# alshai/Big-BWT

Measured on AMD Instinct MI355X. Metric: input MB/s to .bwt (bit-exact vs ref), higher is better.
Workload: dtype u8; 1 GPU; BASELINE configs[2]: 64x mutated yeast-shaped FASTA (~0.79 GB), -w 10 -p 100, BWT + -s -e sampled SA; bytes_per_gpu=787308470, w=10, p=100, flags=6, phrases=16409159, words=921010, dict_bytes=79900101, parallelism=1 GPU

## Files before the change

big-bwt_amd/csrc/api_fm.hip:

```cpp
#include <algorithm>
#include <memory>
#include <utility>
#include <vector>
#include "api.hpp"

using namespace pfp;

struct pfp_fm {
  pfp::FmIndex f;
};

namespace {

template <class F>
int dev_call(pfp_fm *fm, F &&body, bool wait = true) {
  pfp_ctx *c = fm->f.c;
  PFP_TRY_DEV(c)
  body();
  if (wait) sync(c);
  return PFP_OK;
  PFP_CATCH(c)
}

template <class T>
T *hand_out(DBuf<T> &b) { return std::exchange(b.p, nullptr); }

template <class F>
int build_call(pfp_ctx *c, pfp_fm **out, F &&build) {
  *out = nullptr;
  PFP_TRY_DEV(c)
  auto fm = std::make_unique<pfp_fm>();
  build(fm->f);
  *out = fm.release();
  return PFP_OK;
  PFP_CATCH(c)
}

uint64_t pattern_bytes(const uint8_t *pat, const uint64_t *pat_off, uint64_t npat) {
  if (!npat) return 0;
  for (uint64_t p = 0; p < npat; p++)
    PFP_REQUIRE(pat_off[p] <= pat_off[p + 1], PFP_EINVAL, "pattern offsets decrease at pattern " + std::to_string(p));
  PFP_REQUIRE(pat || !pat_off[npat], PFP_EINVAL, "no pattern bytes");
  return pat_off[npat];
}

struct HostPatterns {
  DBuf<uint8_t> pat;
  DBuf<uint64_t> off;
// ... 906 lines not shown
```

big-bwt_amd/csrc/chain.hip:

```cpp
#include "chain.hpp"

using namespace pfp;

namespace pfp {

__global__ void occ_lex_kernel(uint32_t d, const uint32_t *__restrict__ lexrank, const uint32_t *__restrict__ wocc,
                               uint32_t *__restrict__ occ_lex, uint32_t *__restrict__ word_at_rank) {
  uint32_t j = BID * blockDim.x + threadIdx.x;
  if (j >= d) return;
  uint32_t r = lexrank[j];
  occ_lex[r] = wocc[j];
  if (word_at_rank) word_at_rank[r] = j;
}
__global__ void parse_sym_kernel(uint64_t P, const uint32_t *__restrict__ pid, const uint32_t *__restrict__ lexrank,
                                 uint32_t *__restrict__ sym) {
  uint64_t k = (uint64_t)BID * blockDim.x + threadIdx.x;
  if (k < P) sym[k] = lexrank[pid[k]] + 1;
}
__global__ __launch_bounds__(256) void dict_permute_kernel(uint32_t d, const uint32_t *__restrict__ word_at_rank,
                                                           const uint64_t *__restrict__ woff,
                                                           const uint32_t *__restrict__ wlen,
                                                           const uint8_t *__restrict__ src,
                                                           const uint64_t *__restrict__ doff, uint8_t *__restrict__ dst) {
  uint64_t t = (uint64_t)BID * 256 + threadIdx.x;
// ... 76 lines not shown
    st.sa_rounds_parse = ch.pb.rounds;
    if (c->debug) validate_parse_bwt(c, ch.pb);
  }
  {
    PhaseTimer t(c, &st.ms_merge);
    BwtOutputs &bo = ch.out;
    if ((flags & PFP_FLAG_SA) && !d_sa) { ch.sa_own.alloc(c, ch.n_used + 1); d_sa = ch.sa_own.p; }
    bo.d_bwt = d_bwt; bo.d_sa = d_sa;
    with_width(ch.ord.wide, [&](auto tag) {
      using I = decltype(tag);
      merge_bwt<I>(c, ch.D, ch.ix, ch.ord.get<I>(), ch.pb, ch.occ_lex.p, MergeOpts::whole(w, flags, ch.n_used + 1), bo);
    });
    st.hard_groups = bo.hard_groups; st.hard_chars = bo.hard_chars;
    st.hard_big_groups = bo.hard_big_groups; st.hard_max_chars = bo.hard_max_chars; st.hard_max_members = bo.hard_max_members;
    st.hard_minor_groups = bo.hard_minor_groups; st.hard_minor_chars = bo.hard_minor_chars;
  }
  sync(c);
  st.ms_total = std::chrono::duration<double, std::milli>(std::chrono::steady_clock::now() - t0).count();
  *n_used = ch.n_used;
}

template <class Sink>
static void emit_outputs(pfp_ctx *c, const uint8_t *d_bwt, const SaView &d_sa, uint64_t n_out, int flags, Sink &&sink) {
  sink("bwt", d_bwt, n_out);
  if (flags & PFP_FLAG_SA) {
    uint64_t cnt = n_out - 1;
    DBuf<uint8_t> packed(c, cnt * 5 + 16);
    PFP_REQUIRE(d_sa.dense, PFP_EINVAL, "full SA output without the SA values");
    pack5_dev(c, d_sa.dense + 1, cnt, packed.p);
    sink("sa", packed.p, cnt * 5);
    sync(c);
  }
  if (flags & PFP_FLAG_SSA) {
    DBuf<uint8_t> pairs;
    uint64_t k = sample_runs_dev(c, d_bwt, d_sa, n_out, false, pairs);
    sink("ssa", pairs.p, k * 10);
    sync(c);
  }
  if (flags & PFP_FLAG_ESA) {
    DBuf<uint8_t> pairs;
    uint64_t k = sample_runs_dev(c, d_bwt, d_sa, n_out, true, pairs);
    sink("esa", pairs.p, k * 10);
    sync(c);
  }
  sync(c);
}
void fetch_outputs(pfp_ctx *c, const uint8_t *d_bwt, const SaView &d_sa, uint64_t n_out, int flags, pfp_bwt_result *out) {
  emit_outputs(c, d_bwt, d_sa, n_out, flags, [&](const char *name, const uint8_t *d, uint64_t bytes) {
    uint8_t *h = fetch_bytes(c, d, bytes);
    if (name[0] == 'b') { out->bwt = h; out->bwt_size = bytes; }
    else if (name[0] == 's' && name[1] == 'a') { out->sa = h; out->sa_bytes = bytes; }
    else if (name[0] == 's') { out->ssa = h; out->ssa_bytes = bytes; }
    else { out->esa = h; out->esa_bytes = bytes; }
  });
}

}

static bool trace_host() { static const bool on = getenv("PFP_TRACE_HOST") != nullptr; return on; }
static std::chrono::steady_clock::time_point now() { return std::chrono::steady_clock::now(); }
static double ms(std::chrono::steady_clock::time_point a, std::chrono::steady_clock::time_point b) { return std::chrono::duration<double, std::milli>(b - a).count(); }

template <class Stage>
static int bigbwt_to_files(pfp_ctx *c, uint64_t n, int w, uint64_t p, int flags, const char *base, uint64_t out_bytes[4], Stage &&stage) {
  PFP_TRY_DEV(c)
  check_args(w, p, flags);
  const auto t0 = now();
  join_background(c);
  MappedOut m_bwt, m_sa;
  const bool map_bwt = m_bwt.start(c, std::string(base) + ".bwt", n + 1);
  const bool map_sa = (flags & PFP_FLAG_SA) && n && m_sa.start(c, std::string(base) + ".sa", n * 5);
  Chain ch;
  stage(ch.tx);
  if (trace_host()) sync(c);
  const auto t1 = now();
  DBuf<uint8_t> d_bwt(c, n + 1 + 16);
  uint64_t used = 0;
  run_chain_dev(c, ch, n, w, p, flags, d_bwt.p, nullptr, &used);
  const auto t2 = now();
  uint64_t sizes[4] = {0, 0, 0, 0};
  int n_mapped = 0;
  emit_outputs(c, d_bwt.p, sa_view(ch.out), used + 1, flags, [&](const char *name, const uint8_t *d, uint64_t bytes) {
    sizes[name[0] == 'b' ? 0 : (name[1] == 'a' ? 1 : (name[0] == 's' ? 2 : 3))] = bytes;
    if (trace_host()) fprintf(stderr, "[pfp]   %.1f ms after the chain: .%s (%.2f GB) is on the device\n", ms(t2, now()), name, bytes / 1e9);
    MappedOut *mo = name[0] == 'b' ? (map_bwt ? &m_bwt : nullptr) : (name[0] == 's' && name[1] == 'a' && name[2] == 0 ? (map_sa ? &m_sa : nullptr) : nullptr);
    MappedOut late;
    if (!mo && late.start(c, std::string(base) + "." + name, bytes)) mo = &late;
    if (mo && mo->active() && bytes <= mo->bytes) {
      if (mo->write(c, d, bytes)) {
        n_mapped++;
        if (mo != &m_bwt) mo->finish(c, bytes);
        return;
      }
      mo->abandon(false);
    } else if (mo && mo->active()) mo->abandon(false);
    write_dev_file(c, std::string(base) + "." + name, 0, d, bytes, true);
  });
  if (trace_host()) fprintf(stderr, "[pfp]   %.1f ms after the chain: the other files are written\n", ms(t2, now()));
  if (m_bwt.active()) m_bwt.finish(c, sizes[0]);
  if (m_sa.active()) m_sa.abandon(true);
  if (trace_host())
    fprintf(stderr, "[pfp] file to files: text in %.1f ms, chain %.1f ms (first call: the pool is cold), files out %.1f ms%s\n", ms(t0, t1), ms(t1, t2),
            ms(t2, now()), n_mapped ? (std::string(" (") + std::to_string(n_mapped) + " of them straight into the files' mapped pages)").c_str() : "");
  if (out_bytes) memcpy(out_bytes, sizes, sizeof sizes);
  return PFP_OK;
// ... 68 lines not shown
  uint64_t used = 0;
  run_chain_dev(c, ch, n, w, p, flags, d_bwt.p, nullptr, &used);
  const auto t2 = now();
  fetch_outputs(c, d_bwt.p, sa_view(ch.out), used + 1, flags, out);
  if (trace_host())
    fprintf(stderr, "[pfp] host boundary: text in %.1f ms, chain %.1f ms, outputs out %.1f ms (%.2f GB in, %.2f GB out)\n", ms(t0, t1), ms(t1, t2),
            ms(t2, now()), n / 1e9, (out->bwt_size + out->sa_bytes + out->ssa_bytes + out->esa_bytes) / 1e9);
  return PFP_OK;
  PFP_CATCH(c)
}

int pfp_bigbwt_formats_dev(pfp_ctx *c, const void *d_text, uint64_t n, int w, uint64_t p, int flags, void *d_bwt,
                           void *d_out[3], uint64_t out_bytes[3], uint64_t *n_used) {
  if (!c || (!d_text && n) || !d_bwt || !d_out || !out_bytes) return PFP_EINVAL;
  for (int k = 0; k < 3; k++) { d_out[k] = nullptr; out_bytes[k] = 0; }
  PFP_TRY_DEV(c)
  check_args(w, p, flags);
  PFP_REQUIRE(((uintptr_t)d_bwt & 15) == 0, PFP_EINVAL, "d_bwt must be 16-byte aligned");
  Chain ch;
  ch.tx.stage(c, d_text, true, n, w);
  uint64_t used = 0;
  run_chain_dev(c, ch, n, w, p, flags, (uint8_t *)d_bwt, nullptr, &used);
  if (n_used) *n_used = used;
  emit_outputs(c, (const uint8_t *)d_bwt, sa_view(ch.out), used + 1, flags, [&](const char *name, const uint8_t *d, uint64_t bytes) {
    if (name[0] == 'b') return;
    const int k = name[1] == 'a' ? 0 : (name[0] == 's' ? 1 : 2);
    hipError_t e = hipSuccess;
    void *q = c->pool.get(bytes ? bytes : 1, &e, __FILE__, __LINE__);
    if (!q) throw Error(PFP_ENOMEM, std::string("device allocation of an output buffer failed: ") + hipGetErrorString(e));
    PFP_HIP(hipMemcpyAsync(q, d, bytes, hipMemcpyDeviceToDevice, c->stream));
    d_out[k] = q; out_bytes[k] = bytes;
  });
  sync(c);
  return PFP_OK;
  PFP_CATCH(c)
}

int pfp_bigbwt_files(pfp_ctx *c, const uint8_t *text, uint64_t n, int w, uint64_t p, int flags, const char *base,
                     uint64_t out_bytes[4]) {
  if (!c || (!text && n) || !base) return PFP_EINVAL;
  return bigbwt_to_files(c, n, w, p, flags, base, out_bytes, [&](StagedText &tx) { tx.stage(c, text, false, n, w); });
}
int pfp_bigbwt_fd(pfp_ctx *c, int fd, uint64_t file_offset, uint64_t n, int w, uint64_t p, int flags, const char *base,
                  uint64_t out_bytes[4]) {
  if (!c || fd < 0 || !base) return PFP_EINVAL;
  return bigbwt_to_files(c, n, w, p, flags, base, out_bytes, [&](StagedText &tx) { tx.stage_fd(c, fd, file_offset, n, w); });
}

}
```

big-bwt_amd/csrc/common.hpp:

```cpp
#pragma once
#include <hip/hip_runtime.h>
#include <cstdint>
#include <cstdio>
#include <cstring>
#include <stdexcept>
#include <string>
#include <vector>
#include <chrono>
#include <map>
#include <thread>
#include "../../include/pfpgpu.h"

struct K1Scratch; struct DistState;
namespace pfp {
struct StagedText;

constexpr uint8_t kDollar = 2, kEndOfWord = 1, kEndOfDict = 0;
constexpr uint32_t kPrime = 1999999973u;

struct Error : std::runtime_error {
  int code;
  Error(int c, const std::string &m) : std::runtime_error(m), code(c) {}
};

#define PFP_HIP(expr)                                                                     \
  do {                                                                                    \
    hipError_t e__ = (expr);                                                              \
    if (e__ != hipSuccess)                                                                \
      throw ::pfp::Error(PFP_EHIP, std::string(#expr) + ": " + hipGetErrorString(e__) +   \
                                       " (" + __FILE__ + ":" + std::to_string(__LINE__) + ")"); \
  } while (0)

#define PFP_REQUIRE(cond, code, msg)                       \
// ... 214 lines not shown
  DBuf(DBuf &&o) noexcept { *this = std::move(o); }
  DBuf &operator=(DBuf &&o) noexcept {
    if (this != &o) { release(); p = o.p; n = o.n; ctx = o.ctx; o.p = nullptr; o.n = 0; }
    return *this;
  }
  ~DBuf() { release(); }
  void alloc(pfp_ctx *c, size_t count, const char *file = __builtin_FILE(), int line = __builtin_LINE()) {
    release();
    ctx = c; n = count;
    size_t bytes = (count ? count : 1) * sizeof(T);
    if (!c->pool.debug) bytes = (bytes + 511) & ~size_t(511);
    hipError_t e;
    p = (T *)c->pool.get(bytes, &e, file, line);
    if (!p)
      throw Error(e == hipErrorOutOfMemory ? PFP_ENOMEM : PFP_EHIP,
                  std::string("hipMalloc(") + std::to_string(bytes) + "): " + hipGetErrorString(e));
  }
  void release() {
    if (p) { ctx->pool.put(p); p = nullptr; n = 0; }
  }
  void zero() { PFP_HIP(hipMemsetAsync(p, 0, n * sizeof(T), ctx->stream)); }
  size_t bytes() const { return n * sizeof(T); }
};

template <class T>
inline void alloc_counts(pfp_ctx *c, DBuf<T> &b, size_t n, size_t pad = 1, const char *file = __builtin_FILE(), int line = __builtin_LINE()) {
  b.alloc(c, n + pad, file, line);
  PFP_HIP(hipMemsetAsync(b.p + n, 0, sizeof(T), c->stream));
}

template <class T>
inline void d2h(pfp_ctx *c, T *dst, const T *src, size_t count) {
  PFP_HIP(hipMemcpyAsync(dst, src, count * sizeof(T), hipMemcpyDeviceToHost, c->stream));
}
template <class T>
inline void h2d(pfp_ctx *c, T *dst, const T *src, size_t count) {
  PFP_HIP(hipMemcpyAsync(dst, src, count * sizeof(T), hipMemcpyHostToDevice, c->stream));
}
inline void sync(pfp_ctx *c) { c->n_syncs++; PFP_HIP(hipStreamSynchronize(c->stream)); }

template <class T>
inline T read_scalar(pfp_ctx *c, const T *dptr) {
  static_assert(sizeof(T) <= 8, "scalar");
  PFP_HIP(hipMemcpyAsync(c->h_scalars, dptr, sizeof(T), hipMemcpyDeviceToHost, c->stream));
  sync(c);
  T v;
// ... 31 lines not shown
```

big-bwt_amd/csrc/kernels.hpp:

```cpp
#pragma once
#include "common.hpp"
#include "wordview.hpp"

namespace pfp {

struct StagedText {
  static constexpr size_t kFront = 64, kBack = 128;
  DBuf<uint8_t> buf;
  uint64_t n = 0;
  int w = 0;
  const uint8_t *tbase() const { return buf.p + kFront; }
  const uint8_t *tprime() const { return buf.p + kFront - 1; }
  void stage(pfp_ctx *c, const void *src, bool src_on_device, uint64_t n_, int w_);
  void stage_fd(pfp_ctx *c, int fd, uint64_t file_off, uint64_t n_, int w_);
  void restage_tail(pfp_ctx *c, uint64_t new_n, int w_) const;
};

struct KRParams {
  static constexpr uint32_t kMaxExtra = 32;
  uint32_t negpw, pinv, pshift, plimit;
  float fdens = 1.0f;
  uint32_t fthr_nom = 0, fauto = 0;
  uint32_t fast = 0, fseed = 0, fthr = 0;
  uint32_t nextra;
  uint64_t bloom;
  uint32_t extra[kMaxExtra];
};
KRParams make_kr_params(int w, uint64_t p);
KRParams make_fast_params(pfp_ctx *c, const StagedText &tx, uint64_t n, int w, uint64_t p);
KRParams make_fast_params_host(const uint8_t *first_window, int w, uint64_t p, double density_setting, double *density_used);
KRParams params_from_plan(int w, uint64_t p, const uint64_t plan[4]);
struct CutSample { DBuf<uint8_t> nominal; DBuf<uint64_t> hashes; uint64_t ns = 0, counted = 0; };
void classify_cuts(pfp_ctx *c, const StagedText &tx, int w, const DBuf<uint64_t> &d_ends, uint64_t ne, const KRParams &kp, uint64_t min_end,
                   CutSample &out);
bool sample_says_dense(pfp_ctx *c, const uint64_t *d_sorted, uint64_t ns, uint64_t p, uint64_t counts[2] = nullptr);
uint64_t keep_nominal_cuts(pfp_ctx *c, DBuf<uint64_t> &d_ends, uint64_t ne, const DBuf<uint8_t> &nominal);
uint32_t window_hash_host(const uint8_t *win, int w, uint32_t seed);
void scan_flags(pfp_ctx *c, const uint8_t *tbase, uint64_t n, int w, uint64_t p, uint16_t *flags16,
                uint32_t *block_counts, unsigned long long *first_bad, const KRParams *kp_override = nullptr);
uint64_t scan_text(pfp_ctx *c, const StagedText &tx, uint64_t n, int w, uint64_t p, DBuf<uint64_t> &d_ends,
                   uint64_t *n_used, const KRParams *kp_override = nullptr);
uint32_t propose_extra_triggers(pfp_ctx *c, const StagedText &tx, uint64_t n_used, int w, uint64_t max_phrase,
                                const DBuf<uint64_t> &d_ends, uint64_t ne, KRParams &kp);
struct ScanReport {
  KRParams first{}, kp{};
  bool chose = false, dense = false, kr_fallback = false;
  uint64_t sampled = 0, kept = 0, distinct = 0, singles = 0;
  std::vector<uint64_t> dense_ends;
  std::vector<uint8_t> nominal;
};
uint64_t scan_text_adaptive(pfp_ctx *c, const StagedText &tx, uint64_t n, int w, uint64_t p, uint64_t max_phrase,
                            DBuf<uint64_t> &d_ends, uint64_t *n_used, uint32_t *n_extra, ScanReport *rep = nullptr);

struct Dictionary {
  uint64_t P = 0;
  uint64_t d = 0;
  uint64_t dsize = 0;
  DBuf<uint8_t> bytes;
  DBuf<uint64_t> woff;
  DBuf<uint32_t> wlen;
  DBuf<uint32_t> wocc;
  DBuf<uint32_t> pid;
  DBuf<uint8_t> last;
  DBuf<uint64_t> sai;
// ... 329 lines not shown
```

big-bwt_amd/csrc/scan.hip:

```cpp
#include "kernels.hpp"
#include "prims.hpp"
#include "devutil.hpp"

namespace pfp {

constexpr uint32_t kBarrettM = 2305843040u;
static_assert((uint64_t)kBarrettM * kPrime <= (1ull << 62), "barrett");
static_assert((uint64_t)(kBarrettM + 1ull) * kPrime > (1ull << 62), "barrett");

template <int S>
__device__ __forceinline__ uint32_t kr_reduce(uint64_t T) {
  uint32_t xs = (uint32_t)(T >> S);
  uint32_t qhat = __umulhi(xs, kBarrettM) >> (30 - S);
  uint32_t r = (uint32_t)T - qhat * kPrime;
  uint32_t r2 = r - kPrime;
  return r < r2 ? r : r2;
}

constexpr uint32_t kB48 = 140737u;
static_assert((uint64_t)kB48 * kPrime <= (1ull << 48) && (uint64_t)(kB48 + 1) * kPrime > (1ull << 48), "barrett48");
__device__ __forceinline__ uint32_t kr_reduce40(uint32_t lo, uint32_t hi) {
  const uint32_t a = __builtin_amdgcn_alignbit(hi, lo, 16) & 0xFFFFFFu;
  const uint32_t qhat = (uint32_t)(((uint64_t)a * (uint64_t)kB48) >> 32) & 0x3FFu;
  const uint32_t prod = __umul24(qhat, kPrime & 0xFFFFu) + (__umul24(qhat, kPrime >> 16) << 16);
// ... 112 lines not shown
template <int W>
__global__ __launch_bounds__(256) void kr_flag_kernel(const uint8_t *__restrict__ tbase, uint64_t n, KRParams kp,
                                                      uint16_t *__restrict__ flags16,
                                                      uint32_t *__restrict__ block_counts,
                                                      unsigned long long *__restrict__ first_bad) {
  const uint64_t c = (uint64_t)BID * 256 + threadIdx.x;
  const uint64_t pos0 = c * 16;
  uint32_t mask = 0;
  if (pos0 < n) {
    mask = kr_mask16<W>(tbase, pos0, n, kp, first_bad);
    flags16[c] = (uint16_t)mask;
  }
  uint32_t cnt = __popc(mask);
#pragma unroll
  for (int off = 32; off > 0; off >>= 1) cnt += __shfl_down(cnt, off, 64);
  __shared__ uint32_t wsum[4];
  if ((threadIdx.x & 63) == 0) wsum[threadIdx.x >> 6] = cnt;
  __syncthreads();
  if (threadIdx.x == 0 && (uint64_t)BID * 4096 < n) block_counts[BID] = wsum[0] + wsum[1] + wsum[2] + wsum[3];
}

constexpr unsigned long long kTagAgg = 1ull << 62, kTagPre = 2ull << 62, kTagMask = 3ull << 62;
constexpr int kScanChunks = 16;
template <int W, bool FAST>
__global__ __launch_bounds__(256) void kr_scan_kernel(const uint8_t *__restrict__ tbase, uint64_t n, KRParams kp, uint64_t ntiles,
                                                      unsigned int *__restrict__ ticket, unsigned long long *__restrict__ state,
                                                      uint64_t *__restrict__ ends, uint64_t cap,
                                                      unsigned long long *__restrict__ first_bad) {
  __shared__ uint32_t wsum[kScanChunks][4];
  __shared__ unsigned int s_tile;
  __shared__ unsigned long long s_excl;
  if (threadIdx.x == 0) s_tile = atomicAdd(ticket, 1u);
  __syncthreads();
  const uint64_t tile = s_tile;
  if (tile >= ntiles) return;
  const int lane = threadIdx.x & 63, wv = threadIdx.x >> 6;
  uint32_t mask[kScanChunks], incl[kScanChunks];
#pragma unroll 1
  for (int j = 0; j < kScanChunks; j++) {
    const uint64_t c0 = (tile * kScanChunks + j) * 4096;
    const uint64_t pos0 = c0 + (uint64_t)threadIdx.x * 16;
    const bool interior = c0 >= 16 && c0 + 4096 <= n;
    mask[j] = pos0 < n ? kr_mask16<W, FAST>(tbase, pos0, n, kp, first_bad, interior) : 0u;
  }
#pragma unroll
  for (int j = 0; j < kScanChunks; j++) {
    const uint32_t v = wave_incl_sum(__popc(mask[j]));
    incl[j] = v;
    if (lane == 63) wsum[j][wv] = v;
  }
  __syncthreads();
// ... 21 lines not shown
      }
      if (lane == 0) __hip_atomic_store(&state[tile], kTagPre | (excl + agg), __ATOMIC_RELAXED, __HIP_MEMORY_SCOPE_AGENT);
    }
    if (lane == 0) s_excl = excl;
  }
  __syncthreads();
  uint64_t chunk_base = s_excl;
#pragma unroll
  for (int j = 0; j < kScanChunks; j++) {
    uint32_t m = mask[j];
    if (m) {
      uint64_t o = chunk_base + (incl[j] - __popc(m));
      for (int q = 0; q < wv; q++) o += wsum[j][q];
      const uint64_t pos0 = ((tile * kScanChunks + j) * 256 + threadIdx.x) * 16;
      while (m) {
        const int b = __ffs(m) - 1;
        m &= m - 1;
        if (o < cap) ends[o] = pos0 + (uint64_t)b;
        o++;
      }
    }
    chunk_base += (uint64_t)wsum[j][0] + wsum[j][1] + wsum[j][2] + wsum[j][3];
  }
}

__global__ __launch_bounds__(256) void kr_flag_generic_kernel(const uint8_t *__restrict__ tbase, uint64_t n, int W,
                                                              KRParams kp, uint16_t *__restrict__ flags16,
                                                              uint32_t *__restrict__ block_counts,
                                                              unsigned long long *__restrict__ first_bad) {
  const uint64_t c = (uint64_t)BID * 256 + threadIdx.x;
  const uint64_t pos0 = c * 16;
  uint32_t mask = 0;
  if (pos0 < n) {
    for (int k = 0; k < 16; k++)
      if (pos0 + k < n && tbase[pos0 + k] <= 2) { atomicMin(first_bad, (unsigned long long)(pos0 + k)); break; }
    uint32_t h = 0;
    if (pos0 + 1 >= (uint64_t)W) {
      for (int k = 0; k < W; k++) h = kr_reduce<8>(((uint64_t)h << 8) | tbase[pos0 - (W - 1) + k]);
      if (kr_divides(h, kp)) mask |= 1u;
    }
    for (int j = 1; j < 16; j++) {
      uint64_t pos = pos0 + j;
      if (pos + 1 < (uint64_t)W) continue;
      if (pos + 1 == (uint64_t)W) {
        h = 0;
        for (int k = 0; k < W; k++) h = kr_reduce<8>(((uint64_t)h << 8) | tbase[k]);
// ... 139 lines not shown
  hipLaunchKernelGGL(kr_flag_kernel<W>, gdim(nblocks), gdim(256), 0, c->stream, tbase, n, kp, flags16, bc, fb);
}

void scan_flags(pfp_ctx *c, const uint8_t *tbase, uint64_t n, int w, uint64_t p, uint16_t *flags16,
                uint32_t *block_counts, unsigned long long *first_bad, const KRParams *kp_override) {
  KRParams kp = kp_override ? *kp_override : make_kr_params(w, p);
  uint64_t nchunks = cdiv64(n, 16);
  int nblocks = (int)cdiv64(nchunks, 256);
  if (nblocks == 0) return;
  KScope ks(c, "pfp::kr_flag_kernel", n + n / 8);
  switch (w) {
#define CASE(W) case W: launch_flag<W>(c, nblocks, tbase, n, kp, flags16, block_counts, first_bad); break;
    CASE(4) CASE(5) CASE(6) CASE(7) CASE(8) CASE(9) CASE(10) CASE(11) CASE(12) CASE(13) CASE(14) CASE(15) CASE(16) CASE(17)
#undef CASE
    default:
      hipLaunchKernelGGL(kr_flag_generic_kernel, gdim(nblocks), gdim(256), 0, c->stream, tbase, n, w, kp, flags16,
                         block_counts, first_bad);
  }
  PFP_HIP(hipGetLastError());
}

template <int W>
static void launch_scan(pfp_ctx *c, uint64_t ntiles, const uint8_t *tbase, uint64_t n, const KRParams &kp, unsigned int *ticket,
                        unsigned long long *state, uint64_t *ends, uint64_t cap, unsigned long long *fb) {
  if (kp.fast) hipLaunchKernelGGL((kr_scan_kernel<W, true>), gdim(ntiles), gdim(256), 0, c->stream, tbase, n, kp, ntiles, ticket, state, ends, cap, fb);
  else hipLaunchKernelGGL((kr_scan_kernel<W, false>), gdim(ntiles), gdim(256), 0, c->stream, tbase, n, kp, ntiles, ticket, state, ends, cap, fb);
}

uint64_t scan_text(pfp_ctx *c, const StagedText &tx, uint64_t n, int w, uint64_t p, DBuf<uint64_t> &d_ends,
                   uint64_t *n_used, const KRParams *kp_override) {
  PFP_REQUIRE(w >= 1 && w <= 4096, PFP_EINVAL, "window size out of range");
  uint64_t cur_n = n;
  uint64_t cap_hint = 0;
  for (int attempt = 0; attempt < 4; attempt++) {
    uint64_t nchunks = cdiv64(cur_n, 16);
    int nblocks = (int)cdiv64(nchunks, 256);
    *n_used = cur_n;
    if (nblocks == 0) { d_ends.alloc(c, 1); return 0; }
    DBuf<unsigned long long> fbad(c, 1);
    PFP_HIP(hipMemsetAsync(fbad.p, 0xff, 8, c->stream));
    if (w >= 4 && w <= 17) {
      const KRParams kp = kp_override ? *kp_override : make_kr_params(w, p);
      const uint64_t ntiles = cdiv64((uint64_t)nblocks, kScanChunks);
      const uint64_t expect = (uint64_t)((double)(cur_n / (p ? p : 1)) * (kp.fast && kp.fdens > 1.0f ? (double)kp.fdens : 1.0));
      const uint64_t cap = cap_hint ? cap_hint : std::min<uint64_t>(cur_n, expect * 4 + 65536);
      d_ends.alloc(c, cap + 1);
      DBuf<unsigned long long> state(c, ntiles);
      DBuf<unsigned int> ticket(c, 1);
      state.zero(); ticket.zero();
      {
        KScope ks(c, "pfp::kr_scan_kernel", cur_n + 8 * std::min<uint64_t>(cap, expect));
        switch (w) {
#define CASE(W) case W: launch_scan<W>(c, ntiles, tx.tbase(), cur_n, kp, ticket.p, state.p, d_ends.p, cap, fbad.p); break;
          CASE(4) CASE(5) CASE(6) CASE(7) CASE(8) CASE(9) CASE(10) CASE(11) CASE(12) CASE(13) CASE(14) CASE(15) CASE(16) CASE(17)
#undef CASE
        }
        PFP_HIP(hipGetLastError());
      }
      PFP_HIP(hipMemcpyAsync(c->h_scalars, state.p + (ntiles - 1), 8, hipMemcpyDeviceToHost, c->stream));
      PFP_HIP(hipMemcpyAsync(c->h_scalars + 1, fbad.p, 8, hipMemcpyDeviceToHost, c->stream));
      sync(c);
      const uint64_t total = c->h_scalars[0] & ~kTagMask;
      const uint64_t fb = c->h_scalars[1];
      if (fb < cur_n) {
        PFP_REQUIRE(cur_n == n, PFP_EHIP, "scan: special byte after truncation");
        cur_n = fb;
        tx.restage_tail(c, cur_n, w);
        cap_hint = 0;
        continue;
      }
      if (total > cap) { cap_hint = total; continue; }
      return total;
    }
    DBuf<uint16_t> flags16(c, nchunks);
    DBuf<uint32_t> bcnt(c, (size_t)nblocks + 1), boff(c, (size_t)nblocks + 1);
    PFP_HIP(hipMemsetAsync(bcnt.p + nblocks, 0, 4, c->stream));
    scan_flags(c, tx.tbase(), cur_n, w, p, flags16.p, bcnt.p, fbad.p, kp_override);
    exclusive_sum_u32(c, bcnt.p, boff.p, (size_t)nblocks + 1);
    PFP_HIP(hipMemcpyAsync(c->h_scalars, boff.p + nblocks, 4, hipMemcpyDeviceToHost, c->stream));
    PFP_HIP(hipMemcpyAsync(c->h_scalars + 1, fbad.p, 8, hipMemcpyDeviceToHost, c->stream));
    sync(c);
    uint32_t total; memcpy(&total, c->h_scalars, 4);
    uint64_t fb = c->h_scalars[1];
    if (fb < cur_n) {
      PFP_REQUIRE(cur_n == n, PFP_EHIP, "scan: special byte after truncation");
      cur_n = fb;
      tx.restage_tail(c, cur_n, w);
      continue;
    }
    d_ends.alloc(c, (size_t)total + 1);
    KScope ks(c, "pfp::kr_compact_kernel", nchunks * 2 + (uint64_t)total * 8);
    if (total)
      hipLaunchKernelGGL(kr_compact_kernel, gdim(nblocks), gdim(256), 0, c->stream, flags16.p, nchunks, boff.p, d_ends.p);
    PFP_HIP(hipGetLastError());
// ... 49 lines not shown
    sync(c);
    uint64_t h = 0;
    for (int k = 0; k < w; k++) h = (h * 256 + fw[k]) % 1999999973ull;
    h_first = kp.fast ? fast_hash_bytes(fw.data(), w) + kp.fseed : (uint32_t)h;
  }
  uint32_t added = 0;
  for (uint32_t q = 0; q < take; q++) {
    const uint32_t *cand = hv.data() + (size_t)q * kCand;
    uint32_t best = 0, best_mult = kCand + 1;
    for (uint32_t x = 0; x < kCand; x++) {
      uint32_t mult = 0;
      if (cand[x] == h_first) continue;
      for (uint32_t y = 0; y < kCand; y++) mult += cand[y] == cand[x];
      if (mult < best_mult) { best_mult = mult; best = cand[x]; }
    }
    if (best_mult > 4) continue;
    bool dup = false;
    for (uint32_t z = 0; z < kp.nextra; z++) dup |= kp.extra[z] == best;
    if (!dup) { kp.extra[kp.nextra++] = best; kp.bloom |= 1ull << (best & 63); added++; }
  }
  return added;
}

constexpr uint64_t kSampleSlots = 1024;
__global__ __launch_bounds__(256) void classify_ends_kernel(const uint8_t *__restrict__ tbase, const uint64_t *__restrict__ ends, uint64_t ne,
                                                            int w, uint32_t seed, uint32_t thr_nom, uint32_t thr_sample, uint64_t min_end,
                                                            uint8_t *__restrict__ nominal, uint64_t *__restrict__ sample_hash,
                                                            uint64_t slot_cap, unsigned long long *__restrict__ slot_n) {
  const uint64_t k = (uint64_t)BID * blockDim.x + threadIdx.x;
  bool smp = false;
  uint64_t e = 0;
  if (k < ne) {
    e = ends[k];
    const uint32_t x = (fast_hash_bytes(tbase + e - (uint64_t)(w - 1), w) + seed) * kFastK;
    nominal[k] = x < thr_nom ? 1 : 0;
    smp = x < thr_sample && e >= min_end;
  }
  const unsigned long long m = __ballot(smp);
  if (!m) return;
  const int lane = threadIdx.x & 63;
  const uint64_t slot = BID % kSampleSlots;
  unsigned long long base = 0;
  if (lane == __ffsll((long long)m) - 1) base = atomicAdd(&slot_n[slot], (unsigned long long)__popcll(m));
  base = __shfl(base, __ffsll((long long)m) - 1, 64);
  if (!smp) return;
  uint64_t at = base + (uint64_t)__popcll(m & ((1ull << lane) - 1ull));
  if (at >= slot_cap) return;
  at += slot * slot_cap;
  const uint8_t *q = tbase + e - 63;
  uint64_t h = 0x9E3779B97F4A7C15ull;
#pragma unroll
  for (int j = 0; j < 8; j++) h = fmix64(h ^ ld8u(q + 8 * j)) + 0x632BE59BD9B4E019ull * (uint64_t)(j + 1);
  sample_hash[at] = h;
}
__global__ void count_distinct_kernel(const uint64_t *__restrict__ sorted, uint64_t ns, unsigned long long *__restrict__ out) {
  const uint64_t k = (uint64_t)BID * blockDim.x + threadIdx.x;
  const bool head = k < ns && (k == 0 || sorted[k] != sorted[k - 1]);
  const bool single = head && (k + 1 == ns || sorted[k + 1] != sorted[k]);
  const unsigned long long m = __ballot(head), m1 = __ballot(single);
  if ((threadIdx.x & 63) == 0 && m) { atomicAdd(out, (unsigned long long)__popcll(m)); if (m1) atomicAdd(out + 1, (unsigned long long)__popcll(m1)); }
}
__global__ void gather_ends_kernel(const uint64_t *__restrict__ ends, const uint32_t *__restrict__ idx, uint64_t cnt, uint64_t *__restrict__ out) {
  const uint64_t k = (uint64_t)BID * blockDim.x + threadIdx.x;
  if (k < cnt) out[k] = ends[idx[k]];
}
void classify_cuts(pfp_ctx *c, const StagedText &tx, int w, const DBuf<uint64_t> &d_ends, uint64_t ne, const KRParams &kp, uint64_t min_end,
                   CutSample &out) {
  PFP_REQUIRE(ne < 0xFFFFFFFFull, PFP_ELIMIT, "more than 2^32 - 2 phrases (bwtparse.c:93)");
  out.nominal.alloc(c, ne + 16);
  DBuf<uint8_t> &nominal = out.nominal;
  PFP_HIP(hipMemsetAsync(nominal.p + ne, 0, 16, c->stream));
  const uint64_t slot_cap = (ne / 8 + kSampleSlots - 1) / kSampleSlots + 64, scap = slot_cap * kSampleSlots;
  DBuf<uint64_t> h(c, scap);
  DBuf<unsigned long long> sn(c, kSampleSlots);
  PFP_HIP(hipMemsetAsync(h.p, 0xff, scap * 8, c->stream));
  sn.zero();
  hipLaunchKernelGGL(classify_ends_kernel, gdim(cdiv(ne, 256)), gdim(256), 0, c->stream, tx.tbase(), d_ends.p, ne, w, kp.fseed, kp.fthr_nom,
                     kp.fthr_nom / 16u, min_end, nominal.p, h.p, slot_cap, sn.p);
  std::vector<unsigned long long> hsn(kSampleSlots);
  PFP_HIP(hipMemcpyAsync(hsn.data(), sn.p, kSampleSlots * 8, hipMemcpyDeviceToHost, c->stream));
  sync(c);
  uint64_t ns = 0, counted = 0;
  for (unsigned long long v : hsn) { ns += std::min<uint64_t>(v, slot_cap); counted += v; }
  out.ns = ns; out.counted = counted;
  out.hashes.alloc(c, scap);
  sort_keys_raw(c, h.p, out.hashes.p, scap, 0, 64);
}
bool sample_says_dense(pfp_ctx *c, const uint64_t *d_sorted, uint64_t ns, uint64_t p, uint64_t counts[2]) {
  if (counts) counts[0] = counts[1] = 0;
  if (ns < 1024 && !(counts && ns)) return false;
  DBuf<unsigned long long> nd(c, 2);
  nd.zero();
  hipLaunchKernelGGL(count_distinct_kernel, gdim(cdiv(ns, 256)), gdim(256), 0, c->stream, d_sorted, ns, nd.p);
  PFP_HIP(hipMemcpyAsync(c->h_scalars, nd.p, 16, hipMemcpyDeviceToHost, c->stream));
  sync(c);
  const uint64_t distinct = c->h_scalars[0], singles = c->h_scalars[1], loci = distinct - singles;
  if (counts) { counts[0] = distinct; counts[1] = singles; }
  if (ns < 1024) return false;
  return loci >= 64 && singles * 2 <= ns && singles * p >= loci * 64;
}
uint64_t keep_nominal_cuts(pfp_ctx *c, DBuf<uint64_t> &d_ends, uint64_t ne, const DBuf<uint8_t> &nominal) {
  const uint64_t n1 = count_flags(c, nominal.p, ne);
  DBuf<uint64_t> keep(c, n1 + 1), cnt(c, 1);
  DBuf<uint32_t> idx(c, n1 + 1);
  select_index<uint32_t>(c, nominal.p, idx.p, cnt.p, ne);
  if (n1) hipLaunchKernelGGL(gather_ends_kernel, gdim(cdiv(n1, 256)), gdim(256), 0, c->stream, d_ends.p, idx.p, n1, keep.p);
  PFP_HIP(hipGetLastError());
  d_ends = std::move(keep);
  return n1;
}
static uint64_t choose_parse_density(pfp_ctx *c, const StagedText &tx, int w, uint64_t p, DBuf<uint64_t> &d_ends, uint64_t ne, KRParams &kp, bool *dense,
                                     ScanReport *rep) {
  CutSample cs;
  classify_cuts(c, tx, w, d_ends, ne, kp, 0, cs);
  uint64_t counts[2] = {0, 0};
  *dense = sample_says_dense(c, cs.hashes.p, cs.ns, p, rep ? counts : nullptr);
  if (rep) {
    rep->chose = true; rep->dense = *dense;
    rep->sampled = cs.counted; rep->kept = cs.ns; rep->distinct = counts[0]; rep->singles = counts[1];
    rep->dense_ends.resize(ne); rep->nominal.resize(ne);
    d2h(c, rep->dense_ends.data(), d_ends.p, ne);
    d2h(c, rep->nominal.data(), cs.nominal.p, ne);
    sync(c);
  }
  if (*dense) return ne;
  kp.fthr = kp.fthr_nom;
  return keep_nominal_cuts(c, d_ends, ne, cs.nominal);
}

uint64_t scan_text_adaptive(pfp_ctx *c, const StagedText &tx, uint64_t n, int w, uint64_t p, uint64_t max_phrase,
                            DBuf<uint64_t> &d_ends, uint64_t *n_used, uint32_t *n_extra, ScanReport *rep) {
  KRParams kp = c->fast_triggers ? make_fast_params(c, tx, n, w, p) : make_kr_params(w, p);
  *n_extra = 0;
  if (rep) { *rep = ScanReport(); rep->first = kp; }
  uint64_t ne = scan_text(c, tx, n, w, p, d_ends, n_used, &kp);
  c->stats.parse_density = kp.fast ? (c->parse_density > 0 ? c->parse_density : 1.0) : 1.0;
  if (kp.fast && kp.fauto && ne > 0) {
    bool dense = false;
    ne = choose_parse_density(c, tx, w, p, d_ends, ne, kp, &dense, rep);
    c->stats.parse_density = dense ? (double)kp.fdens : 1.0;
  }
  if (kp.fast && ne == 0) {
    kp = make_kr_params(w, p);
    ne = scan_text(c, tx, n, w, p, d_ends, n_used, &kp);
    c->stats.parse_density = 1.0;
    if (rep) rep->kr_fallback = true;
  }
  for (int iter = 0; iter < 4 && max_phrase; iter++) {
    if (!propose_extra_triggers(c, tx, *n_used, w, max_phrase, d_ends, ne, kp)) break;
    ne = scan_text(c, tx, *n_used, w, p, d_ends, n_used, &kp);
  }
  *n_extra = kp.nextra;
  if (rep) rep->kp = kp;
  return ne;
}

}
```

Measured before the change: 28760 MB/s.

## Fuse cut classification into the scan kernel and hand out SA buffers without copies

Cut classification (nominal flag and sampled context positions) now runs as an epilogue of the fast scan kernel, so a separate classify_ends pass over all cuts is no longer needed. Context hashes for the sampled cuts are then computed in a small dedicated kernel. count_distinct is tiled so each block issues fewer atomics, and the device-output path hands over the SA/sampled buffers directly instead of allocating and copying. The scan kernel gains extra work and register pressure in the classify variant, and the sampling order now depends on tile slots.

```diff
diff --git a/big-bwt_amd/csrc/api_fm.hip b/big-bwt_amd/csrc/api_fm.hip
--- a/big-bwt_amd/csrc/api_fm.hip
+++ b/big-bwt_amd/csrc/api_fm.hip
@@ -21,9 +21,6 @@
   return PFP_OK;
   PFP_CATCH(c)
 }
-
-template <class T>
-T *hand_out(DBuf<T> &b) { return std::exchange(b.p, nullptr); }
 
 template <class F>
 int build_call(pfp_ctx *c, pfp_fm **out, F &&build) {
diff --git a/big-bwt_amd/csrc/chain.hip b/big-bwt_amd/csrc/chain.hip
--- a/big-bwt_amd/csrc/chain.hip
+++ b/big-bwt_amd/csrc/chain.hip
@@ -122,31 +122,31 @@
 
 template <class Sink>
 static void emit_outputs(pfp_ctx *c, const uint8_t *d_bwt, const SaView &d_sa, uint64_t n_out, int flags, Sink &&sink) {
-  sink("bwt", d_bwt, n_out);
+  sink("bwt", d_bwt, n_out, nullptr);
   if (flags & PFP_FLAG_SA) {
     uint64_t cnt = n_out - 1;
     DBuf<uint8_t> packed(c, cnt * 5 + 16);
     PFP_REQUIRE(d_sa.dense, PFP_EINVAL, "full SA output without the SA values");
     pack5_dev(c, d_sa.dense + 1, cnt, packed.p);
-    sink("sa", packed.p, cnt * 5);
+    sink("sa", packed.p, cnt * 5, &packed);
     sync(c);
   }
   if (flags & PFP_FLAG_SSA) {
     DBuf<uint8_t> pairs;
     uint64_t k = sample_runs_dev(c, d_bwt, d_sa, n_out, false, pairs);
-    sink("ssa", pairs.p, k * 10);
+    sink("ssa", pairs.p, k * 10, &pairs);
     sync(c);
   }
   if (flags & PFP_FLAG_ESA) {
     DBuf<uint8_t> pairs;
     uint64_t k = sample_runs_dev(c, d_bwt, d_sa, n_out, true, pairs);
-    sink("esa", pairs.p, k * 10);
+    sink("esa", pairs.p, k * 10, &pairs);
     sync(c);
   }
   sync(c);
 }
 void fetch_outputs(pfp_ctx *c, const uint8_t *d_bwt, const SaView &d_sa, uint64_t n_out, int flags, pfp_bwt_result *out) {
-  emit_outputs(c, d_bwt, d_sa, n_out, flags, [&](const char *name, const uint8_t *d, uint64_t bytes) {
+  emit_outputs(c, d_bwt, d_sa, n_out, flags, [&](const char *name, const uint8_t *d, uint64_t bytes, DBuf<uint8_t> *) {
     uint8_t *h = fetch_bytes(c, d, bytes);
     if (name[0] == 'b') { out->bwt = h; out->bwt_size = bytes; }
     else if (name[0] == 's' && name[1] == 'a') { out->sa = h; out->sa_bytes = bytes; }
@@ -180,7 +180,7 @@
   const auto t2 = now();
   uint64_t sizes[4] = {0, 0, 0, 0};
   int n_mapped = 0;
-  emit_outputs(c, d_bwt.p, sa_view(ch.out), used + 1, flags, [&](const char *name, const uint8_t *d, uint64_t bytes) {
+  emit_outputs(c, d_bwt.p, sa_view(ch.out), used + 1, flags, [&](const char *name, const uint8_t *d, uint64_t bytes, DBuf<uint8_t> *) {
     sizes[name[0] == 'b' ? 0 : (name[1] == 'a' ? 1 : (name[0] == 's' ? 2 : 3))] = bytes;
     if (trace_host()) fprintf(stderr, "[pfp]   %.1f ms after the chain: .%s (%.2f GB) is on the device\n", ms(t2, now()), name, bytes / 1e9);
     MappedOut *mo = name[0] == 'b' ? (map_bwt ? &m_bwt : nullptr) : (name[0] == 's' && name[1] == 'a' && name[2] == 0 ? (map_sa ? &m_sa : nullptr) : nullptr);
@@ -295,14 +295,10 @@
   uint64_t used = 0;
   run_chain_dev(c, ch, n, w, p, flags, (uint8_t *)d_bwt, nullptr, &used);
   if (n_used) *n_used = used;
-  emit_outputs(c, (const uint8_t *)d_bwt, sa_view(ch.out), used + 1, flags, [&](const char *name, const uint8_t *d, uint64_t bytes) {
+  emit_outputs(c, (const uint8_t *)d_bwt, sa_view(ch.out), used + 1, flags, [&](const char *name, const uint8_t *, uint64_t bytes, DBuf<uint8_t> *buf) {
     if (name[0] == 'b') return;
     const int k = name[1] == 'a' ? 0 : (name[0] == 's' ? 1 : 2);
-    hipError_t e = hipSuccess;
-    void *q = c->pool.get(bytes ? bytes : 1, &e, __FILE__, __LINE__);
-    if (!q) throw Error(PFP_ENOMEM, std::string("device allocation of an output buffer failed: ") + hipGetErrorString(e));
-    PFP_HIP(hipMemcpyAsync(q, d, bytes, hipMemcpyDeviceToDevice, c->stream));
-    d_out[k] = q; out_bytes[k] = bytes;
+    d_out[k] = hand_out(*buf); out_bytes[k] = bytes;
   });
   sync(c);
   return PFP_OK;
diff --git a/big-bwt_amd/csrc/common.hpp b/big-bwt_amd/csrc/common.hpp
--- a/big-bwt_amd/csrc/common.hpp
+++ b/big-bwt_amd/csrc/common.hpp
@@ -9,6 +9,7 @@
 #include <chrono>
 #include <map>
 #include <thread>
+#include <utility>
 #include "../../include/pfpgpu.h"
 
 struct K1Scratch; struct DistState;
@@ -269,6 +270,8 @@
   void zero() { PFP_HIP(hipMemsetAsync(p, 0, n * sizeof(T), ctx->stream)); }
   size_t bytes() const { return n * sizeof(T); }
 };
+template <class T>
+inline T *hand_out(DBuf<T> &b) { return std::exchange(b.p, nullptr); }
 
 template <class T>
 inline void alloc_counts(pfp_ctx *c, DBuf<T> &b, size_t n, size_t pad = 1, const char *file = __builtin_FILE(), int line = __builtin_LINE()) {
diff --git a/big-bwt_amd/csrc/kernels.hpp b/big-bwt_amd/csrc/kernels.hpp
--- a/big-bwt_amd/csrc/kernels.hpp
+++ b/big-bwt_amd/csrc/kernels.hpp
@@ -39,7 +39,7 @@
 void scan_flags(pfp_ctx *c, const uint8_t *tbase, uint64_t n, int w, uint64_t p, uint16_t *flags16,
                 uint32_t *block_counts, unsigned long long *first_bad, const KRParams *kp_override = nullptr);
 uint64_t scan_text(pfp_ctx *c, const StagedText &tx, uint64_t n, int w, uint64_t p, DBuf<uint64_t> &d_ends,
-                   uint64_t *n_used, const KRParams *kp_override = nullptr);
+                   uint64_t *n_used, const KRParams *kp_override = nullptr, CutSample *classify = nullptr);
 uint32_t propose_extra_triggers(pfp_ctx *c, const StagedText &tx, uint64_t n_used, int w, uint64_t max_phrase,
                                 const DBuf<uint64_t> &d_ends, uint64_t ne, KRParams &kp);
 struct ScanReport {
diff --git a/big-bwt_amd/csrc/scan.hip b/big-bwt_amd/csrc/scan.hip
--- a/big-bwt_amd/csrc/scan.hip
+++ b/big-bwt_amd/csrc/scan.hip
@@ -158,11 +158,30 @@
 
 constexpr unsigned long long kTagAgg = 1ull << 62, kTagPre = 2ull << 62, kTagMask = 3ull << 62;
 constexpr int kScanChunks = 16;
-template <int W, bool FAST>
+template <int W>
+__device__ __forceinline__ uint32_t fast_x_at(const uint8_t *__restrict__ tbase, uint64_t e, uint32_t seed) {
+  const uint4 v = ld16u(tbase + e - 15);
+  const uint32_t d[4] = {v.w, v.z, v.y, v.x};
+  constexpr int nq = (W + 3) / 4;
+  uint32_t h = seed;
+#pragma unroll
+  for (int q = 0; q < nq && q < 4; q++) h = __builtin_amdgcn_udot4(d[q], fast_mvec(W, q), h, false);
+  if constexpr (nq > 4) h = __builtin_amdgcn_udot4((uint32_t)tbase[e - 16] << 24, fast_mvec(W, 4), h, false);
+  return h * kFastK;
+}
+struct ScanClassify {
+  uint8_t *nominal;
+  uint64_t *sample_pos;
+  unsigned long long *slot_n;
+  uint64_t slot_cap;
+  uint32_t nslots, thr_sample;
+};
+template <int W, bool FAST, bool CLS = false>
 __global__ __launch_bounds__(256) void kr_scan_kernel(const uint8_t *__restrict__ tbase, uint64_t n, KRParams kp, uint64_t ntiles,
                                                       unsigned int *__restrict__ ticket, unsigned long long *__restrict__ state,
                                                       uint64_t *__restrict__ ends, uint64_t cap,
-                                                      unsigned long long *__restrict__ first_bad) {
+                                                      unsigned long long *__restrict__ first_bad, ScanClassify cls) {
+  static_assert(FAST || !CLS, "the cuts are classified by the window hash");
   __shared__ uint32_t wsum[kScanChunks][4];
   __shared__ unsigned int s_tile;
   __shared__ unsigned long long s_excl;
@@ -230,6 +249,55 @@
     }
     chunk_base += (uint64_t)wsum[j][0] + wsum[j][1] + wsum[j][2] + wsum[j][3];
   }
+  if constexpr (CLS) {
+    __syncthreads();
+    const uint64_t first = s_excl, last = chunk_base < cap ? chunk_base : cap;
+    unsigned long long *slot_n = cls.slot_n + tile % cls.nslots;
+    uint64_t *list = cls.sample_pos + (tile % cls.nslots) * cls.slot_cap;
+    for (uint64_t k0 = first + (uint64_t)wv * 64; k0 < last; k0 += 256) {
+      const uint64_t k = k0 + (uint64_t)lane;
+      bool smp = false;
+      uint64_t e = 0;
+      if (k < last) {
+        e = __hip_atomic_load(&ends[k], __ATOMIC_RELAXED, __HIP_MEMORY_SCOPE_AGENT);
+        const uint32_t x = fast_x_at<W>(tbase, e, kp.fseed);
+        cls.nominal[k] = x < kp.fthr_nom ? 1 : 0;
+        smp = x < cls.thr_sample;
+      }
+      const unsigned long long m = __ballot(smp);
+      if (!m) continue;
+      const int leader = __ffsll((long long)m) - 1;
+      unsigned long long base = 0;
+      if (lane == leader) base = atomicAdd(slot_n, (unsigned long long)__popcll(m));
+      base = __shfl(base, leader, 64);
+      const uint64_t at = base + (uint64_t)__popcll(m & ((1ull << lane) - 1ull));
+      if (smp && at < cls.slot_cap) list[at] = e;
+    }
+  }
+}
+
+constexpr uint64_t kSampleSlots = 1024;
+__device__ __forceinline__ uint64_t context_hash(const uint8_t *__restrict__ tbase, uint64_t e) {
+  const uint8_t *q = tbase + e - 63;
+  uint64_t h = 0x9E3779B97F4A7C15ull;
+#pragma unroll
+  for (int j = 0; j < 8; j++) h = fmix64(h ^ ld8u(q + 8 * j)) + 0x632BE59BD9B4E019ull * (uint64_t)(j + 1);
+  return h;
+}
+__global__ __launch_bounds__(256) void sample_context_kernel(const uint8_t *__restrict__ tbase, const uint64_t *__restrict__ sample_pos,
+                                                             const unsigned long long *__restrict__ slot_n, uint32_t nslots, uint64_t slot_cap,
+                                                             uint32_t bps, uint64_t *__restrict__ out) {
+  __shared__ unsigned long long ws[4];
+  const uint64_t slot = BID / bps;
+  if (slot >= nslots) return;
+  unsigned long long before = 0;
+  for (uint64_t s = threadIdx.x; s < slot; s += 256) before += slot_n[s] < slot_cap ? slot_n[s] : slot_cap;
+  for (int o = 32; o > 0; o >>= 1) before += __shfl_down(before, o, 64);
+  if ((threadIdx.x & 63) == 0) ws[threadIdx.x >> 6] = before;
+  __syncthreads();
+  before = ws[0] + ws[1] + ws[2] + ws[3];
+  const uint64_t i = (BID % bps) * 256 + threadIdx.x, cnt = slot_n[slot] < slot_cap ? slot_n[slot] : slot_cap;
+  if (i < cnt) out[before + i] = context_hash(tbase, sample_pos[slot * slot_cap + i]);
 }
 
 __global__ __launch_bounds__(256) void kr_flag_generic_kernel(const uint8_t *__restrict__ tbase, uint64_t n, int W,
@@ -415,14 +483,17 @@
 
 template <int W>
 static void launch_scan(pfp_ctx *c, uint64_t ntiles, const uint8_t *tbase, uint64_t n, const KRParams &kp, unsigned int *ticket,
-                        unsigned long long *state, uint64_t *ends, uint64_t cap, unsigned long long *fb) {
-  if (kp.fast) hipLaunchKernelGGL((kr_scan_kernel<W, true>), gdim(ntiles), gdim(256), 0, c->stream, tbase, n, kp, ntiles, ticket, state, ends, cap, fb);
-  else hipLaunchKernelGGL((kr_scan_kernel<W, false>), gdim(ntiles), gdim(256), 0, c->stream, tbase, n, kp, ntiles, ticket, state, ends, cap, fb);
+                        unsigned long long *state, uint64_t *ends, uint64_t cap, unsigned long long *fb, const ScanClassify *cls) {
+  if (cls) hipLaunchKernelGGL((kr_scan_kernel<W, true, true>), gdim(ntiles), gdim(256), 0, c->stream, tbase, n, kp, ntiles, ticket, state, ends, cap, fb, *cls);
+  else if (kp.fast) hipLaunchKernelGGL((kr_scan_kernel<W, true>), gdim(ntiles), gdim(256), 0, c->stream, tbase, n, kp, ntiles, ticket, state, ends, cap, fb, ScanClassify{});
+  else hipLaunchKernelGGL((kr_scan_kernel<W, false>), gdim(ntiles), gdim(256), 0, c->stream, tbase, n, kp, ntiles, ticket, state, ends, cap, fb, ScanClassify{});
 }
 
 uint64_t scan_text(pfp_ctx *c, const StagedText &tx, uint64_t n, int w, uint64_t p, DBuf<uint64_t> &d_ends,
-                   uint64_t *n_used, const KRParams *kp_override) {
+                   uint64_t *n_used, const KRParams *kp_override, CutSample *classify) {
   PFP_REQUIRE(w >= 1 && w <= 4096, PFP_EINVAL, "window size out of range");
+  PFP_REQUIRE(!classify || (w >= 4 && w <= 17 && kp_override && kp_override->fast && !kp_override->nextra), PFP_EINVAL,
+              "scan: only the window hash's own cuts are classified");
   uint64_t cur_n = n;
   uint64_t cap_hint = 0;
   for (int attempt = 0; attempt < 4; attempt++) {
@@ -430,31 +501,44 @@
     int nblocks = (int)cdiv64(nchunks, 256);
     *n_used = cur_n;
     if (nblocks == 0) { d_ends.alloc(c, 1); return 0; }
-    DBuf<unsigned long long> fbad(c, 1);
+    const uint64_t ntiles = cdiv64((uint64_t)nblocks, kScanChunks);
+    const uint32_t nslots = classify ? (uint32_t)std::min<uint64_t>(kSampleSlots, std::max<uint64_t>(1, ntiles / 16)) : 0u;
+    DBuf<unsigned long long> fbad(c, 1 + nslots);
     PFP_HIP(hipMemsetAsync(fbad.p, 0xff, 8, c->stream));
+    if (nslots) PFP_HIP(hipMemsetAsync(fbad.p + 1, 0, (size_t)nslots * 8, c->stream));
     if (w >= 4 && w <= 17) {
       const KRParams kp = kp_override ? *kp_override : make_kr_params(w, p);
-      const uint64_t ntiles = cdiv64((uint64_t)nblocks, kScanChunks);
       const uint64_t expect = (uint64_t)((double)(cur_n / (p ? p : 1)) * (kp.fast && kp.fdens > 1.0f ? (double)kp.fdens : 1.0));
       const uint64_t cap = cap_hint ? cap_hint : std::min<uint64_t>(cur_n, expect * 4 + 65536);
       d_ends.alloc(c, cap + 1);
       DBuf<unsigned long long> state(c, ntiles);
       DBuf<unsigned int> ticket(c, 1);
       state.zero(); ticket.zero();
+      ScanClassify cls{};
+      DBuf<uint64_t> sample_pos;
+      if (classify) {
+        const uint64_t scap = ((cap / 8 + kSampleSlots - 1) / kSampleSlots + 64) * kSampleSlots;
+        cls.slot_cap = cdiv64(scap, nslots);
+        classify->nominal.alloc(c, cap + 16);
+        sample_pos.alloc(c, cls.slot_cap * nslots);
+        cls.nominal = classify->nominal.p; cls.sample_pos = sample_pos.p; cls.slot_n = fbad.p + 1;
+        cls.nslots = nslots; cls.thr_sample = kp.fthr_nom / 16u;
+      }
       {
         KScope ks(c, "pfp::kr_scan_kernel", cur_n + 8 * std::min<uint64_t>(cap, expect));
         switch (w) {
-#define CASE(W) case W: launch_scan<W>(c, ntiles, tx.tbase(), cur_n, kp, ticket.p, state.p, d_ends.p, cap, fbad.p); break;
+#define CASE(W) case W: launch_scan<W>(c, ntiles, tx.tbase(), cur_n, kp, ticket.p, state.p, d_ends.p, cap, fbad.p, classify ? &cls : nullptr); break;
           CASE(4) CASE(5) CASE(6) CASE(7) CASE(8) CASE(9) CASE(10) CASE(11) CASE(12) CASE(13) CASE(14) CASE(15) CASE(16) CASE(17)
 #undef CASE
         }
         PFP_HIP(hipGetLastError());
       }
+      std::vector<unsigned long long> hb(1 + nslots);
       PFP_HIP(hipMemcpyAsync(c->h_scalars, state.p + (ntiles - 1), 8, hipMemcpyDeviceToHost, c->stream));
-      PFP_HIP(hipMemcpyAsync(c->h_scalars + 1, fbad.p, 8, hipMemcpyDeviceToHost, c->stream));
+      PFP_HIP(hipMemcpyAsync(hb.data(), fbad.p, hb.size() * 8, hipMemcpyDeviceToHost, c->stream));
       sync(c);
       const uint64_t total = c->h_scalars[0] & ~kTagMask;
-      const uint64_t fb = c->h_scalars[1];
+      const uint64_t fb = hb[0];
       if (fb < cur_n) {
         PFP_REQUIRE(cur_n == n, PFP_EHIP, "scan: special byte after truncation");
         cur_n = fb;
@@ -463,6 +547,24 @@
         continue;
       }
       if (total > cap) { cap_hint = total; continue; }
+      if (classify) {
+        PFP_HIP(hipMemsetAsync(classify->nominal.p + total, 0, 16, c->stream));
+        uint64_t ns = 0, counted = 0, longest = 0;
+        for (uint32_t s = 0; s < nslots; s++) {
+          const uint64_t kept = std::min<uint64_t>(hb[1 + s], cls.slot_cap);
+          ns += kept; counted += hb[1 + s]; longest = std::max(longest, kept);
+        }
+        classify->ns = ns; classify->counted = counted;
+        classify->hashes.alloc(c, ns);
+        if (ns) {
+          DBuf<uint64_t> h(c, ns);
+          const uint32_t bps = (uint32_t)cdiv64(longest, 256);
+          hipLaunchKernelGGL(sample_context_kernel, gdim((uint64_t)nslots * bps), gdim(256), 0, c->stream, tx.tbase(), sample_pos.p, fbad.p + 1,
+                             nslots, cls.slot_cap, bps, h.p);
+          PFP_HIP(hipGetLastError());
+          sort_keys_raw(c, h.p, classify->hashes.p, ns, 0, 64);
+        }
+      }
       return total;
     }
     DBuf<uint16_t> flags16(c, nchunks);
@@ -558,7 +660,6 @@
   return added;
 }
 
-constexpr uint64_t kSampleSlots = 1024;
 __global__ __launch_bounds__(256) void classify_ends_kernel(const uint8_t *__restrict__ tbase, const uint64_t *__restrict__ ends, uint64_t ne,
                                                             int w, uint32_t seed, uint32_t thr_nom, uint32_t thr_sample, uint64_t min_end,
                                                             uint8_t *__restrict__ nominal, uint64_t *__restrict__ sample_hash,
@@ -583,18 +684,27 @@
   uint64_t at = base + (uint64_t)__popcll(m & ((1ull << lane) - 1ull));
   if (at >= slot_cap) return;
   at += slot * slot_cap;
-  const uint8_t *q = tbase + e - 63;
-  uint64_t h = 0x9E3779B97F4A7C15ull;
-#pragma unroll
-  for (int j = 0; j < 8; j++) h = fmix64(h ^ ld8u(q + 8 * j)) + 0x632BE59BD9B4E019ull * (uint64_t)(j + 1);
-  sample_hash[at] = h;
-}
-__global__ void count_distinct_kernel(const uint64_t *__restrict__ sorted, uint64_t ns, unsigned long long *__restrict__ out) {
-  const uint64_t k = (uint64_t)BID * blockDim.x + threadIdx.x;
-  const bool head = k < ns && (k == 0 || sorted[k] != sorted[k - 1]);
-  const bool single = head && (k + 1 == ns || sorted[k + 1] != sorted[k]);
-  const unsigned long long m = __ballot(head), m1 = __ballot(single);
-  if ((threadIdx.x & 63) == 0 && m) { atomicAdd(out, (unsigned long long)__popcll(m)); if (m1) atomicAdd(out + 1, (unsigned long long)__popcll(m1)); }
+  sample_hash[at] = context_hash(tbase, e);
+}
+constexpr int kDistinctTile = 2048;
+__global__ __launch_bounds__(256) void count_distinct_kernel(const uint64_t *__restrict__ sorted, uint64_t ns, unsigned long long *__restrict__ out) {
+  __shared__ uint32_t ws[2][4];
+  uint32_t heads = 0, singles = 0;
+#pragma unroll
+  for (int r = 0; r < kDistinctTile / 256; r++) {
+    const uint64_t k = (uint64_t)BID * kDistinctTile + (uint64_t)r * 256 + threadIdx.x;
+    const bool head = k < ns && (k == 0 || sorted[k] != sorted[k - 1]);
+    const bool single = head && (k + 1 == ns || sorted[k + 1] != sorted[k]);
+    heads += (uint32_t)__popcll(__ballot(head));
+    singles += (uint32_t)__popcll(__ballot(single));
+  }
+  if ((threadIdx.x & 63) == 0) { ws[0][threadIdx.x >> 6] = heads; ws[1][threadIdx.x >> 6] = singles; }
+  __syncthreads();
+  if (threadIdx.x == 0) {
+    const uint32_t a = ws[0][0] + ws[0][1] + ws[0][2] + ws[0][3], b = ws[1][0] + ws[1][1] + ws[1][2] + ws[1][3];
+    if (a) atomicAdd(out, (unsigned long long)a);
+    if (b) atomicAdd(out + 1, (unsigned long long)b);
+  }
 }
 __global__ void gather_ends_kernel(const uint64_t *__restrict__ ends, const uint32_t *__restrict__ idx, uint64_t cnt, uint64_t *__restrict__ out) {
   const uint64_t k = (uint64_t)BID * blockDim.x + threadIdx.x;
@@ -627,7 +737,7 @@
   if (ns < 1024 && !(counts && ns)) return false;
   DBuf<unsigned long long> nd(c, 2);
   nd.zero();
-  hipLaunchKernelGGL(count_distinct_kernel, gdim(cdiv(ns, 256)), gdim(256), 0, c->stream, d_sorted, ns, nd.p);
+  hipLaunchKernelGGL(count_distinct_kernel, gdim(cdiv64(ns, kDistinctTile)), gdim(256), 0, c->stream, d_sorted, ns, nd.p);
   PFP_HIP(hipMemcpyAsync(c->h_scalars, nd.p, 16, hipMemcpyDeviceToHost, c->stream));
   sync(c);
   const uint64_t distinct = c->h_scalars[0], singles = c->h_scalars[1], loci = distinct - singles;
@@ -645,10 +755,8 @@
   d_ends = std::move(keep);
   return n1;
 }
-static uint64_t choose_parse_density(pfp_ctx *c, const StagedText &tx, int w, uint64_t p, DBuf<uint64_t> &d_ends, uint64_t ne, KRParams &kp, bool *dense,
+static uint64_t choose_parse_density(pfp_ctx *c, uint64_t p, DBuf<uint64_t> &d_ends, uint64_t ne, KRParams &kp, const CutSample &cs, bool *dense,
                                      ScanReport *rep) {
-  CutSample cs;
-  classify_cuts(c, tx, w, d_ends, ne, kp, 0, cs);
   uint64_t counts[2] = {0, 0};
   *dense = sample_says_dense(c, cs.hashes.p, cs.ns, p, rep ? counts : nullptr);
   if (rep) {
@@ -669,13 +777,16 @@
   KRParams kp = c->fast_triggers ? make_fast_params(c, tx, n, w, p) : make_kr_params(w, p);
   *n_extra = 0;
   if (rep) { *rep = ScanReport(); rep->first = kp; }
-  uint64_t ne = scan_text(c, tx, n, w, p, d_ends, n_used, &kp);
+  CutSample cs;
+  const bool choose = kp.fast && kp.fauto;
+  uint64_t ne = scan_text(c, tx, n, w, p, d_ends, n_used, &kp, choose ? &cs : nullptr);
   c->stats.parse_density = kp.fast ? (c->parse_density > 0 ? c->parse_density : 1.0) : 1.0;
-  if (kp.fast && kp.fauto && ne > 0) {
+  if (choose && ne > 0) {
     bool dense = false;
-    ne = choose_parse_density(c, tx, w, p, d_ends, ne, kp, &dense, rep);
+    ne = choose_parse_density(c, p, d_ends, ne, kp, cs, &dense, rep);
     c->stats.parse_density = dense ? (double)kp.fdens : 1.0;
   }
+  cs = CutSample();
   if (kp.fast && ne == 0) {
     kp = make_kr_params(w, p);
     ne = scan_text(c, tx, n, w, p, d_ends, n_used, &kp);
```

After: 29340 MB/s, median of 6. 1.02x the previous value.
